# kisasexypantera94/hpfw

Measured on AMD Instinct MI355X. Metric: hashprints/sec (index) + Hamming matches/sec (search), 30 s@44.1 kHz clips, higher is better.
Workload: dtype f32 (transforms, dB) + int8 digits / int64 sums (projection); 1 GPU; configs[1]: 1000 x 30 s synthetic 44.1 kHz PCM16 clips per GPU, hashprint extraction only (CQT + dB + projection + bit pack), inputs resident in HBM; clips_per_gpu=1000, hashprints_per_clip=2320, parallelism=clips sharded over 1 GPU(s), no collective on this path

## Files before the change

### hpfw_amd/csrc/extract.hip

```cpp
#include "handle.h"

int pass_clips(hpfw_gpu *h, const DevPlan *dp, int64_t n_clips)
{
    const hpfw::HostPlan &p = dp->hp;
    size_t per_clip = (size_t)121 * p.c * 4 + (size_t)64 * std::max(p.n_frames, 1) * 4;
    if (p.bluestein)
        per_clip += 2 * hpfw::bz_plane_bytes(dp->bz, 1) + (size_t)(p.kmax - p.kmin) * 8;
    else
        per_clip += (size_t)hpfw::z_floats_per_clip(p.hq, p.n2) * 4 + (size_t)p.n1 * p.q2w * 8;
    size_t work = 0;
    for (const hpfw::CqClassDev &cd : dp->cls) work = std::max(work, hpfw::cq_big_work_bytes(cd, 1));
    per_clip += work;
    const int64_t fit = std::max<int64_t>(1, (int64_t)(((size_t)24 << 30) / per_clip));
    const int64_t cap = std::min<int64_t>(h->batch, fit), n = std::max<int64_t>(n_clips, 1);
    const int64_t passes = (n + cap - 1) / cap;
    return (int)((n + passes - 1) / passes);
}

int ensure_ws(hpfw_gpu *h, const DevPlan *dp, int nb, int ns)
{
    const hpfw::HostPlan &p = dp->hp;
    size_t work = 0;
    for (const hpfw::CqClassDev &cd : dp->cls) work = std::max(work, hpfw::cq_big_work_bytes(cd, nb));
    if (work) {
// ... 148 lines not shown
#endif
#if defined(HPFW_ROWS_STAMPS)
        dp->rows.stamps = reinterpret_cast<long long *>(g_rows_snap);
#endif
        hpfw::launch_fwd_rows2(dp->rows, dp->rows_out, yp, nb, x, s);
    }
    return check_launch("fwd_rows");
}
}

int run_front(hpfw_gpu *h, DevPlan *dp, const int16_t *d_pcm, int nb, int slot, bool finish_db, hipStream_t s)
{
    using hpfw::cf;
    const hpfw::HostPlan &p = dp->hp;
    cf *x = h->ws[1].as<cf>();
    float *mag = h->ws[2].as<float>() + (size_t)slot * 121 * p.c;
    float *mm = h->ws[4].as<float>() + (size_t)slot * 121 * hpfw::kCqMaxWaves;
    float *clipmax = h->d_clipmax.as<float>() + slot;
    int rc;
    if ((rc = run_forward(h, dp, d_pcm, nb, x, s))) return rc;
    {
        Timed t(h, K_CQ, s);
        int n_lds = 0;
        for (const hpfw::CqClassDev &cd : dp->cls) n_lds += cd.outer ? 0 : 1;
        const bool fork = h->cq_concurrent && n_lds > 1 && nb >= 4;
        Fanout fan(h, s);
        if (fork && (rc = fan.fork(hpfw_gpu::kCqSide))) return rc;
        int turn = 0;
        for (size_t ci = dp->cls.size(); ci-- > 0;) {
            const hpfw::CqClassDev &cd = dp->cls[ci];
            if (cd.outer) {
                hpfw::launch_cq_big_class(dp->cq, cd, x, nb, h->d_cqwork.as<cf>(), mag, mm, h->db_fast ? hpfw::kDbFast : hpfw::kDbSpec, s);
                continue;
            }
            const int lane = fork ? turn++ % (hpfw_gpu::kCqSide + 1) : 0;
            hpfw::launch_cq_class(dp->cq, cd, x, nb, mag, mm, h->db_fast ? hpfw::kDbFast : hpfw::kDbSpec, fan.lane(lane));
        }
        if ((rc = check_launch("cq_chirpz"))) return rc;
    }
    {
        Timed t(h, K_DB, s);
        hpfw::launch_clipmax(mm, clipmax, nb, s);
        if (finish_db) hpfw::launch_db_finish(mag, clipmax, nb, (int64_t)121 * p.c, s);
    }
    return check_launch("db");
}

int q_split(hpfw_gpu *h, int n_shifts, int64_t n_clips, int64_t c, hpfw::QSplit *qs, const hpfw::QSplit **use)
{
    *use = nullptr;
    if (n_shifts || h->q_products != 6 || !h->projection) return 0;
    const int64_t tiles = hpfw::project_q_tiles(n_clips, c);
    if (tiles <= 0) return 0;
    if (int rc = ensure(h->d_q_split, hpfw::project_q_split_bytes(tiles), h)) return rc;
    *qs = {h->d_fq_thr.as<int32_t>(), h->d_q_split.get()};
    *use = qs;
    return 0;
}

namespace {
int run_back(hpfw_gpu *h, DevPlan *dp, const void *images, int n_shifts, int ns, uint64_t *d_hp, hipStream_t s)
{
    const hpfw::HostPlan &p = dp->hp;
    const float *sdb = h->ws[2].as<float>();
    int rc;
    if (h->projection) {
        hpfw::QSplit qs;
        const hpfw::QSplit *split;
        if ((rc = q_split(h, n_shifts, ns, p.c, &qs, &split))) return rc;
        {
            Timed t(h, K_PROJECT, s);
            hpfw::launch_hashprints_q(images, n_shifts, sdb, h->d_clipmax.as<float>(), ns, p.c, d_hp, nullptr, s, split);
        }
        if (split) h->q_last_tiles = hpfw::project_q_tiles(ns, p.c);
        return check_launch("project");
    }
    float *proj = h->ws[3].as<float>();
    {
        Timed t(h, K_PROJECT, s);
        hpfw::launch_project(h->d_fpack.as<float>(), sdb, h->d_clipmax.as<float>(), ns, p.c, proj, s);
    }
    if ((rc = check_launch("project"))) return rc;
    {
        Timed t(h, K_PACK, s);
        hpfw::launch_pack(proj, ns, p.n_frames, d_hp, s);
    }
    return check_launch("delta_pack");
}

constexpr int kBackBatch = 1024;

int check_filters(const hpfw_gpu *h) { return h->has_filters ? 0 : fail(HPFW_E_NOFILTERS, "no filters: call hpfw_gpu_set_filters or hpfw_gpu_learn_filters first"); }

int check_shifts(const int32_t *shifts, int n_shifts)
{
    if (!shifts || n_shifts < 1 || n_shifts > hpfw::kMaxShifts) return fail(HPFW_E_INVALID, "shifts: 1 to 64 values");
    for (int i = 0; i < n_shifts; ++i) {
        if (shifts[i] < -(hpfw::kBins - 1) || shifts[i] > hpfw::kBins - 1) return fail(HPFW_E_INVALID, "shifts: |s| <= 120");
        for (int j = 0; j < i; ++j)
            if (shifts[j] == shifts[i]) return fail(HPFW_E_INVALID, "shifts: values must be distinct");
    }
    return 0;
}

int shift_images(hpfw_gpu *h, const int32_t *shifts, int n_shifts, hipStream_t s)
{
    std::vector<int32_t> want(shifts, shifts + n_shifts);
    if (want == h->shift_images_of) return 0;
// ... 723 lines not shown
```

### hpfw_amd/csrc/handle.h

```cpp
#pragma once
#include <hip/hip_runtime.h>

#include <algorithm>
#include <cstdio>
#include <cstdlib>
#include <cstring>
#include <condition_variable>
#include <chrono>
#include <map>
#include <memory>
#include <mutex>
#include <set>
#include <string>
#include <vector>

#include "../../include/hpfw_gpu.h"
#include "combiner.h"
#include "hip_owned.h"
#include "kernels.h"
#include "legacy_internal.h"
#include "plan.h"

using hpfw::DevBuf, hpfw::Event, hpfw::HostBuf, hpfw::Stream;

int fail(int code, const std::string &msg);

#define HIP_TRY(expr)                                                                                   \
    do {                                                                                                \
        hipError_t e_ = (expr);                                                                         \
        if (e_ != hipSuccess)                                                                           \
            return fail(HPFW_E_HIP, std::string(#expr) + ": " + hipGetErrorString(e_));                 \
    } while (0)

struct DevPlan {
    hpfw_gpu *owner = nullptr;
    std::vector<DevBuf> blocks;
    char *cur = nullptr;
    size_t left = 0;
    char *chunk_base = nullptr;
    std::vector<char> stage;
    std::vector<std::pair<size_t, size_t>> staged;
    hpfw::HostPlan hp;
    hpfw::ColsQArgs cols;
    hpfw::Rows2Out rows_out;
    hpfw::RowsArgs rows;
    hpfw::BzArgs bz;
    hpfw::CqPlanDev cq;
    std::vector<hpfw::CqClassDev> cls;
    size_t bytes = 0;
    uint64_t last_use = 0;
    ~DevPlan();
};

struct PlanTiming;

enum KernelKind { K_ROWS = 0, K_COLS, K_CQ, K_DB, K_PROJECT, K_PACK, K_SCAN, K_TOPK, K_PAIRS, K_FWD, K_COUNT };

struct TimedLaunch {
    int kind;
    Event a, b;
};

struct CallStatus {
    int rc = 0;
    std::string msg;
};

struct hpfw_gpu {
    int device = 0;
    bool has_filters = false;
    std::vector<float> filters;
    DevBuf d_fpack;
    DevBuf d_fq_image;
    DevBuf d_fq_thr, d_q_split;
    int q_products = 6;
    int64_t q_last_tiles = 0;
    int projection = 1;
    struct PlanCache {
        PlanCache();
        ~PlanCache();
        std::multimap<size_t, DevBuf> dev_pool;
        size_t dev_pool_bytes = 0;
        std::map<int64_t, std::unique_ptr<DevPlan>> plans;
        std::mutex host_mtx;
        std::condition_variable host_cv;
        std::map<int64_t, std::unique_ptr<hpfw::HostPlan>> host_ready;
        std::set<int64_t> host_seen;
        size_t plan_bytes = 0;
        uint64_t plan_clock = 0;
        uint64_t idle_clock = 0;
        std::unique_ptr<PlanTiming> plan_timing;
        Stream plan_stream;
        HostBuf pin_ring;
        size_t pin_off = 0;
        Event plan_ev;
        bool plan_ev_pending = false;
    } cache;
    unsigned conventions = 0;
    int batch = 256;
    DevBuf ws[7];
    struct Index {
        DevBuf d_db;
        std::vector<int64_t> db_off{0};
        DevBuf d_db_off;
        bool db_off_dirty = true;
        uint32_t clip_base = 0;
        DevBuf d_best, d_q_off;
        DevBuf d_qa;
        DevBuf d_gk;
        DevBuf d_topk_scratch;
        DevBuf d_shift_hits;
    } index;
    struct Learn {
        DevBuf d_cov;
        DevBuf d_cov_ws;
        DevBuf d_cov_tiles;
        int64_t cov_files = 0;
        std::map<std::vector<int>, DevBuf> cfg_fpack;
        DevBuf d_cfg_proj;
        struct CfgCov {
            DevBuf d_accum;
            DevBuf d_tiles;
            int64_t clips = 0;
        };
        std::map<std::vector<int>, CfgCov> cfg_cov;
        DevBuf d_cfg_cov_ws;
    } learn;
    struct Mel {
// ... 148 lines not shown
```

### hpfw_amd/csrc/handle.hip

```cpp
#include "handle.h"

namespace {
thread_local std::string g_err;

const char *const kKernelNames[K_COUNT] = {"fwd_rows", "fwd_cols", "cq_chirpz", "db",
                                           "project_mfma", "delta_pack", "hamming_scan", "topk", "pcm_pairs", "fwd_span"};
}

int fail(int code, const std::string &msg)
{
    g_err = msg;
    return code;
}

extern "C" {

const char *hpfw_gpu_last_error(void) { return g_err.c_str(); }
void hpfw_internal_set_error(const char *msg) { g_err = msg ? msg : ""; }
const char *hpfw_gpu_version(void) { return "hpfw-gpu 0.1 (gfx950)"; }

int hpfw_gpu_create(int device, hpfw_gpu **out)
{
    if (!out) return fail(HPFW_E_INVALID, "out is NULL");
    *out = nullptr;
    int n = 0;
    HIP_TRY(hipGetDeviceCount(&n));
    if (device < 0 || device >= n) return fail(HPFW_E_INVALID, "no such device");
    HIP_TRY(hipSetDevice(device));
    auto h = std::make_unique<hpfw_gpu>();
    h->device = device;
    if (std::getenv("HPFW_CQ_SERIAL")) h->cq_concurrent = 0;
    if (const char *e = std::getenv("HPFW_FWD_CHUNK")) h->fwd_chunk = std::max(0, atoi(e));
    if (const char *e = std::getenv("HPFW_BZ_CHUNK")) h->bz_chunk = std::max(0, atoi(e));
    if (const char *e = std::getenv("HPFW_COLS_VARIANT")) h->cols_variant = atoi(e);
    if (const char *e = std::getenv("HPFW_PRUNE")) h->prune = (unsigned)std::strtoul(e, nullptr, 0);
    if (const char *e = std::getenv("HPFW_Q_PRODUCTS")) h->q_products = atoi(e) == 9 ? 9 : 6;
    if (const char *e = std::getenv("HPFW_DB_TERM")) h->db_fast = std::strcmp(e, "spec") != 0;
    if (const char *e = std::getenv("HPFW_FWD_STREAMS")) h->fwd_streams = std::min(hpfw_gpu::kCqSide + 1, std::max(1, atoi(e)));
    if (const char *e = std::getenv("HPFW_PROJECTION"))
        h->projection = std::strcmp(e, "f32") == 0 ? 0 : 1;
    if (h->ev0.create(hipEventDefault) != hipSuccess || h->ev1.create(hipEventDefault) != hipSuccess || h->order_ev.create() != hipSuccess ||
        init_plans(h.get()) != hipSuccess)
        return fail(HPFW_E_HIP, "hipEventCreate failed");
    *out = h.release();
    return 0;
}

int hpfw_gpu_device(const hpfw_gpu *h) { return h ? h->device : -1; }

void hpfw_gpu_destroy(hpfw_gpu *h)
{
    if (!h) return;
    (void)hipSetDevice(h->device);
    (void)hipDeviceSynchronize();
    delete h;
}

int hpfw_gpu_set_filters(hpfw_gpu *h, const float *f)
{
    if (!h || !f) return fail(HPFW_E_INVALID, "null argument");
    HIP_TRY(hipSetDevice(h->device));
    std::vector<float> packed((size_t)hpfw::kFilters * hpfw::kFrame);
    hpfw::pack_filters_for_mfma(f, packed.data());
    if (!h->d_fpack) HIP_TRY(h->d_fpack.alloc(packed.size() * 4));
    HIP_TRY(hipMemcpy(h->d_fpack.get(), packed.data(), packed.size() * 4, hipMemcpyHostToDevice));
    std::vector<int8_t> image;
    std::vector<int32_t> fq_thr;
    hpfw::pack_filters_q(f, image, &fq_thr);
    if (!h->d_fq_image) HIP_TRY(h->d_fq_image.alloc(image.size()));
    HIP_TRY(hipMemcpy(h->d_fq_image.get(), image.data(), image.size(), hipMemcpyHostToDevice));
    if (!h->d_fq_thr) HIP_TRY(h->d_fq_thr.alloc(fq_thr.size() * 4));
    HIP_TRY(hipMemcpy(h->d_fq_thr.get(), fq_thr.data(), fq_thr.size() * 4, hipMemcpyHostToDevice));
    h->shift_images_of.clear();
    h->filters.assign(f, f + (size_t)hpfw::kFilters * hpfw::kFrame);
    h->has_filters = true;
    return 0;
}

int hpfw_gpu_get_filters(hpfw_gpu *h, float *out)
{
    if (!h || !out) return fail(HPFW_E_INVALID, "null argument");
    if (!h->has_filters) return fail(HPFW_E_NOFILTERS, "no filters: call hpfw_gpu_set_filters or hpfw_gpu_learn_filters first");
    std::memcpy(out, h->filters.data(), h->filters.size() * sizeof(float));
    return 0;
}

int hpfw_gpu_set_projection(hpfw_gpu *h, int mode)
{
    if (!h || (mode != 0 && mode != 1)) return fail(HPFW_E_INVALID, "projection mode must be 0 (f32 chain) or 1 (fixed point)");
    h->projection = mode;
    return 0;
}

int hpfw_gpu_get_projection(hpfw_gpu *h) { return h ? h->projection : -1; }

int hpfw_gpu_set_conventions(hpfw_gpu *h, unsigned flags)
{
    if (!h || flags > hpfw::kConvAll) return fail(HPFW_E_INVALID, "unknown convention flag");
    HIP_TRY(hipSetDevice(h->device));
    if (flags != h->conventions) {
        HIP_TRY(hipDeviceSynchronize());
        clear_plans(h);
    }
    h->conventions = flags;
    return 0;
}

int hpfw_gpu_set_batch(hpfw_gpu *h, int clips)
{
    if (!h || clips < 0 || clips > 4096) return fail(HPFW_E_INVALID, "batch out of range");
    h->batch = clips == 0 ? 256 : clips;
    return 0;
}

int hpfw_gpu_timer_start(hpfw_gpu *h, void *stream)
{
    if (!h) return fail(HPFW_E_INVALID, "null handle");
    HIP_TRY(hipEventRecord(h->ev0.get(), (hipStream_t)stream));
    return 0;
}

int hpfw_gpu_timer_stop(hpfw_gpu *h, void *stream, float *ms)
{
    if (!h || !ms) return fail(HPFW_E_INVALID, "null argument");
    HIP_TRY(hipEventRecord(h->ev1.get(), (hipStream_t)stream));
// ... 41 lines not shown
```

### hpfw_amd/csrc/k_project_q.hip

```cpp
#include <algorithm>
#include <cmath>
#include <cstdint>
#include <cstdlib>
#include <vector>

#include "kernels.h"

namespace hpfw {

extern __shared__ __align__(16) unsigned char smem_raw[];

typedef int v4i __attribute__((ext_vector_type(4)));
typedef int v16i __attribute__((ext_vector_type(16)));

constexpr int kQThreads = 256;
constexpr int kQTileN = 128;
constexpr int kQCols = kQTileN + kCtx - 1;
constexpr int kQPitch = 160;
constexpr int kQChunks = 8;
constexpr int kQUnit = 48;
constexpr int kQSlabBytes = kQChunks * kQPitch * kQUnit;
constexpr int kQStepBytes = 3 * 64 * 16;
constexpr int kQSteps = 2 * kCtx;
constexpr int kQLdsBytes = kQSlabBytes + kQTileN * 4 * 2;
constexpr float kQScale = 98304.0f;
constexpr int kQCap = 128;
constexpr unsigned kQRedo = 0xffffffffu;
constexpr int kQLdsBytes6 = kQLdsBytes + 16;

__device__ __forceinline__ unsigned q_digit_bytes(int u) { return ((unsigned)u + 0x808080u) ^ 0x808080u; }

__device__ __forceinline__ int q_fixed(float s)
{
    return (int)__builtin_rintf(__builtin_fminf(__builtin_fmaxf(s, -80.0f), 0.0f) * kQScale);
}

template <bool FROM_T, bool SHIFTED, int NP>
__device__ __forceinline__ void hashprint_q_tile(const unsigned t, const v4i *__restrict__ fq_images, const float *__restrict__ sdb,
                                                 const float *__restrict__ tmax, int c, int nhp, int n_tiles_x, uint64_t *__restrict__ hp,
                                                 long long *__restrict__ dbg, int n_images, const int *__restrict__ thr,
                                                 unsigned *__restrict__ counts, unsigned short *__restrict__ seg)
{
    static_assert(NP == 9 || (NP == 6 && !SHIFTED), "six products: the extraction's unshifted image only");
    unsigned char *slab = smem_raw;
    unsigned short *parts = reinterpret_cast<unsigned short *>(smem_raw + kQSlabBytes);
    unsigned *n_open = reinterpret_cast<unsigned *>(smem_raw + kQLdsBytes);
    const int tid = threadIdx.x, lane = tid & 63, wave = tid >> 6;
    const int kg = lane >> 4, cl = lane & 15;
    const int clip = t / n_tiles_x;
    const int n0 = (t - clip * n_tiles_x) * kQTileN;
    if (NP == 6 && tid == 0) *n_open = 0;
#if defined(HPFW_Q_STAMPS)
    long long st[6];
    st[0] = __builtin_amdgcn_s_memtime();
#define Q_STAMP(k) st[k] = __builtin_amdgcn_s_memtime()
#else
#define Q_STAMP(k) ((void)0)
#endif
    const float *S = sdb + (int64_t)clip * kBins * c;
    const float ref = FROM_T ? tmax[clip] : 0.0f;
    const v4i *img = fq_images + (size_t)wave * kQSteps * (kQStepBytes / 16) + lane;
    v4i a[3][3];
#pragma unroll
    for (int d = 0; d < 3; ++d) {
        a[0][d] = img[d * 64];
        a[1][d] = img[(kQStepBytes / 16) + d * 64];
    }
    constexpr int kUnits = (kQChunks * kQCols + kQThreads - 1) / kQThreads;
    unsigned any_digit = 0;
#pragma unroll 1
    for (int r0 = 0; r0 < kUnits; r0 += 2) {
        float va[2][16], vb[2][16];
#pragma unroll
        for (int rr = 0; rr < 2; ++rr) {
            const int unit = tid + (r0 + rr) * kQThreads;
            const int q = unit / kQCols, col = unit - q * kQCols;
            const int gc = n0 + col;
            const bool in = r0 + rr < kUnits && unit < kQChunks * kQCols && gc + kLag < c;
#pragma unroll
            for (int e = 0; e < 16; ++e) {
                const int bin = 16 * q + e;
                const bool ok = in && bin < kBins;
                const unsigned idx = ok ? (unsigned)(bin * c + gc) : 0u;
                va[rr][e] = S[idx];
                vb[rr][e] = S[idx + kLag];
            }
        }
#pragma unroll
        for (int rr = 0; rr < 2; ++rr) {
            const int unit = tid + (r0 + rr) * kQThreads;
            const int q = unit / kQCols, col = unit - q * kQCols;
            const bool in = r0 + rr < kUnits && unit < kQChunks * kQCols && n0 + col + kLag < c;
#pragma unroll
            for (int e = 0; e < 16; ++e) {
                const bool ok = in && 16 * q + e < kBins;
                va[rr][e] = ok ? va[rr][e] : 0.0f;
                vb[rr][e] = ok ? vb[rr][e] : 0.0f;
            }
        }
#pragma unroll
        for (int rr = 0; rr < 2; ++rr) {
            const int unit = tid + (r0 + rr) * kQThreads;
            if (r0 + rr >= kUnits || unit >= kQChunks * kQCols) break;
            const int q = unit / kQCols, col = unit - q * kQCols;
            unsigned w0[4] = {0, 0, 0, 0}, w1[4] = {0, 0, 0, 0}, w2[4] = {0, 0, 0, 0};
#pragma unroll
            for (int e = 0; e < 16; ++e) {
                float xa = va[rr][e], xb = vb[rr][e];
                if (FROM_T) {
                    xa -= ref;
                    xb -= ref;
                }
                const unsigned d = q_digit_bytes(q_fixed(xa) - q_fixed(xb));
                w0[e >> 2] |= (d & 255u) << (8 * (e & 3));
                w1[e >> 2] |= ((d >> 8) & 255u) << (8 * (e & 3));
                w2[e >> 2] |= ((d >> 16) & 255u) << (8 * (e & 3));
            }
            v4i *dst = reinterpret_cast<v4i *>(slab + (size_t)(q * kQPitch + col) * kQUnit);
            dst[0] = v4i{(int)w0[0], (int)w0[1], (int)w0[2], (int)w0[3]};
            dst[1] = v4i{(int)w1[0], (int)w1[1], (int)w1[2], (int)w1[3]};
            dst[2] = v4i{(int)w2[0], (int)w2[1], (int)w2[2], (int)w2[3]};
            if (NP == 6)
                any_digit |= w0[0] | w0[1] | w0[2] | w0[3] | w1[0] | w1[1] | w1[2] | w1[3] | w2[0] | w2[1] | w2[2] | w2[3];
        }
    }
    Q_STAMP(1);
    if (NP == 6) {
        if (!__syncthreads_or((int)(any_digit != 0))) {
            if (tid < kQTileN && n0 + tid < nhp) hp[(int64_t)clip * nhp + n0 + tid] = ~0ull;
            if (tid == 0) counts[t] = 0;
            return;
        }
    } else {
        __syncthreads();
    }
    Q_STAMP(2);
    const int n_tiles = min(8, (nhp - n0 + 15) / 16);
    const unsigned char *bl = slab + (size_t)(kg * kQPitch + cl) * kQUnit;
    int im = 0;
#pragma unroll 1
    do {
        if (SHIFTED && im > 0) {
            __syncthreads();
            img += (size_t)4 * kQSteps * kQStepBytes / 16;
#pragma unroll
            for (int d = 0; d < 3; ++d) {
                a[0][d] = img[d * 64];
                a[1][d] = img[(kQStepBytes / 16) + d * 64];
            }
        }
        v4i acc[8][5];
#pragma unroll
        for (int f = 0; f < 8; ++f)
#pragma unroll
            for (int cls = 0; cls < 5; ++cls) acc[f][cls] = v4i{0, 0, 0, 0};
        auto step = [&](int s, const v4i (&aw)[3]) {
            const unsigned char *bs = bl + (size_t)((4 * (s & 1)) * kQPitch + (s >> 1)) * kQUnit;
            v4i nb0, nb1, nb2;
            {
                const v4i *bu = reinterpret_cast<const v4i *>(bs);
                nb0 = bu[0], nb1 = bu[1], nb2 = bu[2];
            }
#pragma unroll
            for (int f = 0; f < 8; ++f) {
                if (f < n_tiles) {
                    const v4i b0 = nb0, b1 = nb1, b2 = nb2;
                    if (f + 1 < 8) {
                        const v4i *bu = reinterpret_cast<const v4i *>(bs + (size_t)(16 * (f + 1)) * kQUnit);
                        nb0 = bu[0], nb1 = bu[1], nb2 = bu[2];
                    }
                    __builtin_amdgcn_sched_barrier(0);
                    if (NP == 9) {
                        acc[f][0] = __builtin_amdgcn_mfma_i32_16x16x64_i8(aw[0], b0, acc[f][0], 0, 0, 0);
                        acc[f][1] = __builtin_amdgcn_mfma_i32_16x16x64_i8(aw[0], b1, acc[f][1], 0, 0, 0);
                    }
                    acc[f][2] = __builtin_amdgcn_mfma_i32_16x16x64_i8(aw[0], b2, acc[f][2], 0, 0, 0);
                    acc[f][3] = __builtin_amdgcn_mfma_i32_16x16x64_i8(aw[1], b2, acc[f][3], 0, 0, 0);
                    acc[f][4] = __builtin_amdgcn_mfma_i32_16x16x64_i8(aw[2], b2, acc[f][4], 0, 0, 0);
                    if (NP == 9) acc[f][1] = __builtin_amdgcn_mfma_i32_16x16x64_i8(aw[1], b0, acc[f][1], 0, 0, 0);
                    acc[f][2] = __builtin_amdgcn_mfma_i32_16x16x64_i8(aw[1], b1, acc[f][2], 0, 0, 0);
                    acc[f][3] = __builtin_amdgcn_mfma_i32_16x16x64_i8(aw[2], b1, acc[f][3], 0, 0, 0);
                    acc[f][2] = __builtin_amdgcn_mfma_i32_16x16x64_i8(aw[2], b0, acc[f][2], 0, 0, 0);
                }
            }
        };
        auto load_a = [&](int s, v4i (&aw)[3]) {
            if (s < kQSteps) {
#pragma unroll
                for (int d = 0; d < 3; ++d) aw[d] = img[(size_t)s * (kQStepBytes / 16) + d * 64];
            }
        };
        if (n_tiles > 0) {
#pragma unroll 1
            for (int s = 0; s < kQSteps - 1; s += 3) {
                load_a(s + 2, a[2]);
                step(s, a[0]);
                load_a(s + 3, a[0]);
                step(s + 1, a[1]);
                load_a(s + 4, a[1]);
                step(s + 2, a[2]);
            }
            step(kQSteps - 1, a[0]);
        }
        Q_STAMP(3);
        v4i th = v4i{-1, -1, -1, -1};
        if (NP == 6) th = *reinterpret_cast<const v4i *>(thr + 16 * wave + 4 * kg);
#pragma unroll
        for (int f = 0; f < 8; ++f) {
            const int n = n0 + 16 * f + cl;
            (void)n;
            unsigned bits = 0;
#pragma unroll
            for (int reg = 0; reg < 4; ++reg) {
                const int row = 4 * kg + reg;
                long long v = acc[f][4][reg];
#pragma unroll
                for (int cls = 3; cls >= (NP == 9 ? 0 : 2); --cls) v = v * 256 + acc[f][cls][reg];
                bits |= (unsigned)(v >= 0) << (15 - row);
                if (NP == 6 && f < n_tiles && n < nhp && (v < 0 ? -v : v) <= (long long)th[reg]) {
                    const unsigned pos = atomicAdd(n_open, 1u);
                    if (pos < (unsigned)kQCap) seg[(size_t)t * kQCap + pos] = (unsigned short)(((16 * wave + row) << 7) | (16 * f + cl));
                }
#if !defined(HPFW_Q_STAMPS)
                if (!SHIFTED && dbg && f < n_tiles && n < nhp) dbg[((int64_t)clip * kFilters + 16 * wave + row) * nhp + n] = v;
#endif
            }
            bits |= (unsigned)__shfl_xor((int)bits, 16);
            bits |= (unsigned)__shfl_xor((int)bits, 32);
            if (kg == 0) parts[(16 * f + cl) * 4 + wave] = (unsigned short)bits;
        }
        Q_STAMP(4);
        __syncthreads();
        if (tid < kQTileN && n0 + tid < nhp) {
            const unsigned short *p = parts + tid * 4;
            hp[((int64_t)clip * (SHIFTED ? n_images : 1) + im) * nhp + n0 + tid] =
                ((uint64_t)p[0] << 48) | ((uint64_t)p[1] << 32) | ((uint64_t)p[2] << 16) | (uint64_t)p[3];
        }
        if (NP == 6 && tid == 0) counts[t] = *n_open <= (unsigned)kQCap ? *n_open : kQRedo;
    } while (SHIFTED && ++im < n_images);
#if defined(HPFW_Q_STAMPS)
    Q_STAMP(5);
    if (dbg && tid == 0) {
        for (int k = 0; k < 6; ++k) dbg[(int64_t)t * 8 + k] = st[k];
        dbg[(int64_t)t * 8 + 6] = __builtin_amdgcn_s_getreg((15 << 11) | 4);
        dbg[(int64_t)t * 8 + 7] = blockIdx.x;
    }
#endif
}

__device__ __forceinline__ unsigned q_tile_of_workgroup()
{
    const unsigned per_xcd = (gridDim.x + 7) / 8;
    return (blockIdx.x & 7) * per_xcd + (blockIdx.x >> 3);
}

template <bool FROM_T, bool SHIFTED>
__global__ __launch_bounds__(kQThreads, 2) void hashprint_q_kernel(const v4i *__restrict__ fq_images, const float *__restrict__ sdb,
                                                                   const float *__restrict__ tmax, int c, int nhp, int n_tiles_x, int n_clips,
                                                                   uint64_t *__restrict__ hp, long long *__restrict__ dbg, int n_images)
{
    const unsigned t = q_tile_of_workgroup();
    if (t >= (unsigned)(n_tiles_x * n_clips)) return;
    hashprint_q_tile<FROM_T, SHIFTED, 9>(t, fq_images, sdb, tmax, c, nhp, n_tiles_x, hp, dbg, n_images, nullptr, nullptr, nullptr);
}

template <bool FROM_T>
__global__ __launch_bounds__(kQThreads, 2) void hashprint_q6_kernel(const v4i *__restrict__ fq_image, const float *__restrict__ sdb,
                                                                    const float *__restrict__ tmax, int c, int nhp, int n_tiles_x, int n_clips,
                                                                    uint64_t *__restrict__ hp, const int *__restrict__ thr,
                                                                    unsigned *__restrict__ counts, unsigned short *__restrict__ seg)
{
    const unsigned t = q_tile_of_workgroup();
    if (t >= (unsigned)(n_tiles_x * n_clips)) return;
    hashprint_q_tile<FROM_T, false, 6>(t, fq_image, sdb, tmax, c, nhp, n_tiles_x, hp, nullptr, 1, thr, counts, seg);
}

template <bool FROM_T>
__global__ __launch_bounds__(kQThreads, 2) void hashprint_q_fixup_kernel(const v4i *__restrict__ fq_image, const int *__restrict__ fq32,
                                                                         const float *__restrict__ sdb, const float *__restrict__ tmax, int c,
                                                                         int nhp, int n_tiles_x, int n_clips, uint64_t *__restrict__ hp,
                                                                         const unsigned *__restrict__ counts,
                                                                         const unsigned short *__restrict__ seg)
{
    const int lane = threadIdx.x & 63, wave = threadIdx.x >> 6;
    const unsigned total = (unsigned)(n_tiles_x * n_clips);
    for (unsigned t = blockIdx.x; t < total; t += gridDim.x) {
        const unsigned cnt = counts[t];
        if (cnt == 0) continue;
        if (cnt == kQRedo) {
            __syncthreads();
            hashprint_q_tile<FROM_T, false, 9>(t, fq_image, sdb, tmax, c, nhp, n_tiles_x, hp, nullptr, 1, nullptr, nullptr, nullptr);
            continue;
        }
        const int clip = t / n_tiles_x;
        const int n0 = (t - clip * n_tiles_x) * kQTileN;
        const float *S = sdb + (int64_t)clip * kBins * c;
        const float ref = FROM_T ? tmax[clip] : 0.0f;
        for (unsigned e = wave; e < cnt; e += kQThreads / 64) {
            const unsigned entry = seg[(size_t)t * kQCap + e];
            const int r = entry >> 7, n = n0 + (int)(entry & 127u);
            const int *frow = fq32 + r * kFrame;
            long long sum = 0;
#pragma unroll 2
            for (int k = lane; k < kFrame; k += 64) {
                const int bin = k / kCtx, idx = bin * c + n + (k - bin * kCtx);
                float xa = S[idx], xb = S[idx + kLag];
                if (FROM_T) {
                    xa -= ref;
                    xb -= ref;
                }
                sum += (long long)frow[k] * (long long)(q_fixed(xa) - q_fixed(xb));
            }
#pragma unroll
            for (int m = 32; m >= 1; m >>= 1) sum += __shfl_xor(sum, m);
            if (lane == 0) {
                unsigned long long *w = reinterpret_cast<unsigned long long *>(hp + (int64_t)clip * nhp + n);
                const unsigned long long bit = 1ull << (63 - r);
                if (((*w & bit) != 0) != (sum >= 0)) atomicXor(w, bit);
            }
        }
    }
}

__global__ __launch_bounds__(256) void shift_filter_images_kernel(const unsigned char *__restrict__ base, ShiftList shifts,
                                                                  v4i *__restrict__ out)
{
    constexpr int kUnits = 4 * kQSteps * kQStepBytes / 16;
    const int u = blockIdx.x * 256 + threadIdx.x;
    if (u >= kUnits) return;
    const int s = shifts.s[blockIdx.y];
    const int l = u & 63, i = (u >> 6) % 3, ws = u / 192;
    const int step = ws % kQSteps, w = ws / kQSteps, t = step >> 1, p = step & 1;
    unsigned wd[4] = {0, 0, 0, 0};
#pragma unroll
    for (int e = 0; e < 16; ++e) {
        const int b = 64 * p + 16 * (l >> 4) + e, src = b - s;
        if (b < kBins && src >= 0 && src < kBins) {
            const unsigned char v = base[((size_t)w * kQSteps + 2 * t + (src >> 6)) * kQStepBytes + ((size_t)i * 64 + (l & 15) + 16 * ((src >> 4) & 3)) * 16 +
                                         (src & 15)];
            wd[e >> 2] |= (unsigned)v << (8 * (e & 3));
        }
    }
    out[(size_t)blockIdx.y * kUnits + u] = v4i{(int)wd[0], (int)wd[1], (int)wd[2], (int)wd[3]};
}

void pack_filters_q(const float *f, std::vector<int8_t> &image, std::vector<int32_t> *fq_thr)
{
    std::vector<int32_t> fq((size_t)kFilters * kFrame);
    for (int r = 0; r < kFilters; ++r) {
        float m = 0.0f;
        for (int k = 0; k < kFrame; ++k) m = std::fmax(m, std::fabs(f[(size_t)k * kFilters + r]));
        const int e = m > 0.0f ? 21 - std::ilogb(m) : 0;
        for (int k = 0; k < kFrame; ++k) fq[(size_t)r * kFrame + k] = (int32_t)std::rint(std::ldexp(f[(size_t)k * kFilters + r], e));
    }
    if (fq_thr) {
        fq_thr->assign(fq.begin(), fq.end());
        for (int r = 0; r < kFilters; ++r) {
            int64_t s0 = 0, s1 = 0;
            for (int k = 0; k < kFrame; ++k) {
                const int u = fq[(size_t)r * kFrame + k];
                const int d0 = ((u + 128) & 255) - 128, u1 = (u - d0) >> 8, d1 = ((u1 + 128) & 255) - 128;
                s0 += std::abs(d0);
                s1 += std::abs(d1);
            }
            const int64_t lmax = 128 * (s0 + 256 * (s0 + s1));
            fq_thr->push_back(lmax > 0 ? (int32_t)(lmax >> 16) : -1);
        }
    }
    image.assign((size_t)4 * kQSteps * kQStepBytes, 0);
    for (int w = 0; w < 4; ++w)
        for (int t = 0; t < kCtx; ++t)
            for (int p = 0; p < 2; ++p)
                for (int l = 0; l < 64; ++l)
                    for (int e = 0; e < 16; ++e) {
                        const int bin = 64 * p + 16 * (l >> 4) + e;
                        if (bin >= kBins) continue;
                        const int u = fq[(size_t)(16 * w + (l & 15)) * kFrame + bin * kCtx + t];
                        const int d0 = ((u + 128) & 255) - 128, u1 = (u - d0) >> 8, d1 = ((u1 + 128) & 255) - 128, d2 = (u1 - d1) >> 8;
                        const int d[3] = {d0, d1, d2};
                        for (int i = 0; i < 3; ++i)
                            image[((size_t)w * kQSteps + (2 * t + p)) * kQStepBytes + ((size_t)i * 64 + l) * 16 + e] = (int8_t)d[i];
                    }
}

#if defined(HPFW_Q_STAMPS)
static long long *g_q_stamps = nullptr;
extern "C" void hpfw_gpu_debug_set_q_stamps(void *d) { g_q_stamps = static_cast<long long *>(d); }
#endif

size_t project_q_image_bytes() { return (size_t)4 * kQSteps * kQStepBytes; }
size_t project_q_split_bytes(int64_t tiles) { return (size_t)tiles * (4 + (size_t)kQCap * 2); }
int64_t project_q_tiles(int64_t n_clips, int64_t c)
{
    const int64_t nhp = c - (kCtx - 1) - kLag;
    return nhp > 0 ? n_clips * ((nhp + kQTileN - 1) / kQTileN) : 0;
}

void launch_hashprints_q(const void *d_images, int n_shifts, const float *d_db, const float *d_tmax, int n_clips, int c, uint64_t *d_hp,
                         long long *d_dbg, hipStream_t s, const QSplit *split)
{
    static PerDeviceOnce attr_set;
    if (attr_set.need()) {
        for (const void *k : {reinterpret_cast<const void *>(hashprint_q_kernel<true, false>), reinterpret_cast<const void *>(hashprint_q_kernel<false, false>),
                              reinterpret_cast<const void *>(hashprint_q_kernel<true, true>), reinterpret_cast<const void *>(hashprint_q_kernel<false, true>)})
            (void)hipFuncSetAttribute(k, hipFuncAttributeMaxDynamicSharedMemorySize, kQLdsBytes);
        for (const void *k : {reinterpret_cast<const void *>(hashprint_q6_kernel<true>), reinterpret_cast<const void *>(hashprint_q6_kernel<false>),
                              reinterpret_cast<const void *>(hashprint_q_fixup_kernel<true>), reinterpret_cast<const void *>(hashprint_q_fixup_kernel<false>)})
            (void)hipFuncSetAttribute(k, hipFuncAttributeMaxDynamicSharedMemorySize, kQLdsBytes6);
        attr_set.mark();
    }
    const int nhp = c - (kCtx - 1) - kLag;
    if (nhp <= 0 || n_clips <= 0 || n_shifts < 0) return;
#if defined(HPFW_Q_STAMPS)
    if (!d_dbg) d_dbg = g_q_stamps;
#endif
    const int tiles = (nhp + kQTileN - 1) / kQTileN;
    const dim3 grid(8 * (unsigned)(((int64_t)tiles * n_clips + 7) / 8));
    if (split && n_shifts == 0 && !d_dbg) {
        const int *fq32 = split->d_fq_thr, *thr = fq32 + (size_t)kFilters * kFrame;
        unsigned *counts = static_cast<unsigned *>(split->d_work);
        unsigned short *seg = reinterpret_cast<unsigned short *>(counts + (size_t)tiles * n_clips);
        hipLaunchKernelGGL(d_tmax ? hashprint_q6_kernel<true> : hashprint_q6_kernel<false>, grid, dim3(kQThreads), kQLdsBytes6, s,
                           static_cast<const v4i *>(d_images), d_db, d_tmax, c, nhp, tiles, n_clips, d_hp, thr, counts, seg);
        const unsigned fix = (unsigned)std::min<int64_t>((int64_t)tiles * n_clips, 2048);
        hipLaunchKernelGGL(d_tmax ? hashprint_q_fixup_kernel<true> : hashprint_q_fixup_kernel<false>, dim3(fix), dim3(kQThreads), kQLdsBytes6, s,
                           static_cast<const v4i *>(d_images), fq32, d_db, d_tmax, c, nhp, tiles, n_clips, d_hp, counts, seg);
        return;
    }
    auto k = n_shifts > 0 ? (d_tmax ? hashprint_q_kernel<true, true> : hashprint_q_kernel<false, true>)
                          : (d_tmax ? hashprint_q_kernel<true, false> : hashprint_q_kernel<false, false>);
    hipLaunchKernelGGL(k, grid, dim3(kQThreads), kQLdsBytes, s, static_cast<const v4i *>(d_images), d_db, d_tmax, c, nhp, tiles, n_clips,
                       d_hp, d_dbg, n_shifts);
}

void launch_shift_filter_images(const void *d_fq_image, const ShiftList &shifts, void *d_images, hipStream_t s)
{
    constexpr int kUnits = 4 * kQSteps * kQStepBytes / 16;
    hipLaunchKernelGGL(shift_filter_images_kernel, dim3((kUnits + 255) / 256, shifts.n), dim3(256), 0, s,
                       static_cast<const unsigned char *>(d_fq_image), shifts, static_cast<v4i *>(d_images));
}

}
```

### hpfw_amd/csrc/kernels.h

```cpp
#pragma once
#include <cmath>
#include <cstdint>
#include <vector>
#include <atomic>
#include <hip/hip_runtime.h>
#include <stdint.h>

#include "../../include/hpfw_gpu.h"
#include "device_math.h"
#include "fft_lds.h"
#include "fft_rows.h"
#include "streams_plan.h"
#include "xcorr_plan.h"

namespace hpfw {

struct PerDeviceOnce {
    std::atomic<uint64_t> done{0};
    static uint64_t bit()
    {
        int dev = 0;
        (void)hipGetDevice(&dev);
        return 1ull << (dev & 63);
    }
// ... 125 lines not shown
    int kmin, nk;
    int xn1, xw, xq0;
    int64_t xclip;
    unsigned long long xmagic;
    HPFW_DEVICE_MEMBER XsView view(const cf *x, int clip) const { return XsView{x + (int64_t)clip * xclip, xn1, xw, xq0, xmagic}; }
    int c;
    const int *start;
    const int *lg;
    const int64_t *g_off;
    const cf *g;
    const cf *g2;
    const int64_t *g2_off;
    const int *q2a, *nq2;
    const unsigned *nq2_magic;
    int rows_min;
};

struct CqWindowBands {
    double scale[121];
    int hann_den[121];
};
void launch_cq_windows(const CqPlanDev &c, const CqWindowBands &b, int64_t big_m, int lg_max, cf *d_g, hipStream_t s);
void launch_cq_windows_rows(const CqPlanDev &c, int n1, int max_entries, cf *d_g2, hipStream_t s);

void launch_fwd_cols_q(const ColsQArgs &a, const int16_t *d_pcm, int64_t clip_samples, int n_clips, float *d_z, hipStream_t s);
size_t fwd_rows_lds_bytes(const RowsArgs &a);
void launch_fwd_rows2(const RowsArgs &a, const Rows2Out &o, const float *d_z, int n_clips, cf *d_x, hipStream_t s);
void launch_gather_bins(const CqPlanDev &cp, const cf *d_x, int n_clips, cf *d_out, hipStream_t s);
size_t bz_plane_bytes(const BzArgs &bz, int n_clips);
void launch_bz_pack_stages(const BzArgs &bz, const cf *d_tw_n1, float *d_apack1, float *d_apack3, hipStream_t s);
void launch_bz_pack_coefficients(int n1, int k1_first, int k1_count, const cf *d_tw_n1, int n_tiles, float *d_apack, hipStream_t s);
void launch_bz_make_tables(const RowsArgs &rows, const BzArgs &bz, int64_t n, float *d_b, float *d_y, hipStream_t s);
void launch_bz_cols_first(const BzArgs &bz, const int16_t *d_pcm, int64_t n, int n_clips, float *d_out, hipStream_t s);
void launch_bz_rows_both(const RowsArgs &rows, const BzArgs &bz, const float *d_in, int n_clips, float *d_out, hipStream_t s);
void launch_bz_cols_last(const BzArgs &bz, const float *d_in, int n_clips, cf *d_x, hipStream_t s);
constexpr int kCqMaxWaves = 16;
enum DbMode { kDbNone = 0, kDbSpec = 1, kDbFast = 2 };
void launch_cq_class(const CqPlanDev &cp, const CqClassDev &cc, const cf *d_x, int n_clips,
                     float *d_mag, float *d_wavemax, int db_mode, hipStream_t s);
size_t cq_big_work_bytes(const CqClassDev &cc, int n_clips);
void launch_cq_big_class(const CqPlanDev &cp, const CqClassDev &cc, const cf *d_x, int n_clips, cf *d_work, float *d_mag,
                         float *d_wavemax, int db_mode, hipStream_t s);
void launch_clipmax(const float *d_wavemax, float *d_clipmax, int n_clips, hipStream_t s);
void launch_db_finish(float *d_t, const float *d_clipmax, int n_clips, int64_t per_clip, hipStream_t s);
void launch_magmax(const float *d_mag, int n_clips, int c, float *d_wavemax, hipStream_t s);
void launch_db(const float *d_mag, const float *d_wavemax, float *d_clipmax, int n_clips, int64_t per_clip,
               float *d_db, bool fast, hipStream_t s);
void launch_db_term_sweep(uint32_t first, uint64_t count, unsigned long long *d_out, hipStream_t s);
void launch_project(const float *d_fpack, const float *d_db, const float *d_tmax, int n_clips, int c,
                    float *d_proj, hipStream_t s);
void launch_pack(const float *d_proj, int n_clips, int nf, uint64_t *d_hp, hipStream_t s);
size_t project_q_image_bytes();
struct QSplit {
    const int32_t *d_fq_thr;
    void *d_work;
};
size_t project_q_split_bytes(int64_t tiles);
int64_t project_q_tiles(int64_t n_clips, int64_t c);
void pack_filters_q(const float *f_colmajor, std::vector<int8_t> &image, std::vector<int32_t> *fq_thr = nullptr);
void launch_hashprints_q(const void *d_images, int n_shifts, const float *d_db, const float *d_tmax, int n_clips, int c, uint64_t *d_hp,
                         long long *d_dbg, hipStream_t s, const QSplit *split = nullptr);
constexpr int kMaxShifts = 64;
struct ShiftList {
    int n;
    int s[kMaxShifts];
};
void launch_shift_filter_images(const void *d_fq_image, const ShiftList &shifts, void *d_images, hipStream_t s);
constexpr int kMaxTempos = 64;
struct TempoList {
    int n;
    int32_t step[kMaxTempos];
};
inline int32_t tempo_step(float rho) { return (int32_t)std::rint(65536.0 / (double)rho); }
inline int64_t tempo_columns(int64_t c, int32_t step) { return (c - 1) * 65536 / step + 1; }
void launch_tempo_scale(const float *d_db, int n_clips, int64_t c, const TempoList &tl, int64_t ct, float *d_out, hipStream_t s);

struct CfgArgs {
    int rows, context, lag, filters;
    const float *fpack;
};
size_t cfg_fpack_floats(int rows, int context, int filters);
void pack_cfg_filters(int rows, int context, int filters, const float *f_colmajor, float *fpack);
size_t project_cfg_lds_bytes(const CfgArgs &a);
void launch_project_cfg(const CfgArgs &a, const float *d_s, const int *d_cols, int n_clips, int64_t stride, float *d_proj,
                        int64_t proj_stride, hipStream_t s);
void launch_pack_cfg(const CfgArgs &a, const float *d_proj, const int *d_cols, int n_clips, int64_t stride, int64_t proj_stride,
                     void *d_hp, int64_t hp_stride, hipStream_t s);

bool cov_cfg_supported(const CfgArgs &a);
int cov_cfg_tile_count(int kt);
void cov_cfg_tile_list(int kt, int *xy );
size_t cov_cfg_workspace_bytes(const CfgArgs &a, int n_clips);
void launch_cov_cfg(const CfgArgs &a, const float *d_s, const int *d_cols, int n_clips, int64_t stride, const int *d_tiles,
                    float *d_ws, float *d_accum, hipStream_t s);

int cov_tile_count();
void cov_tile_list(int *xy );
size_t cov_workspace_bytes(int n_clips, int c);
void launch_cov(const float *d_db, int n_clips, int c, const int *d_tiles, float *d_ws, float *d_accum, hipStream_t s);
int top_eigenvectors(const float *cov, int n, int m, float *out, double *evals);

void pack_filters_for_mfma(const float *filters_colmajor, float *fpack );

constexpr int kMelFrame = 4410, kMelHop = 441, kMelBins = 2206, kMelBands = 33;
int mel_frames(int64_t n_samples);
size_t mel_work_bytes(int64_t n_samples, int n_clips);
void launch_mel(const RowsArgs &rows, const float *d_win, const float *d_cpack, const int16_t *d_pcm, int64_t n, int n_clips,
                int64_t *d_blk, int *d_pos, int *d_count, float *d_pmax, float *d_work, float *d_out, bool db_fast, hipStream_t s);
void launch_mel_kept_frames(const int16_t *d_pcm, int64_t n, int n_clips, int64_t *d_blk, int *d_pos, int *d_count,
                            int32_t *d_frames, int64_t stride, hipStream_t s);

void launch_xcorr(const int16_t *d_pcm, const XcJob *d_jobs, int64_t n_jobs, const XcItem *d_mfma, int64_t n_mfma,
// ... 66 lines not shown
```

Baseline: 276.8 million hashprints/s.

## Fuse six-product projection fixup into the main kernel using LDS entry list

The six-product quantized projection previously wrote near-threshold entries to a global segment list, and a separate fixup kernel recomputed them. It now keeps the list in LDS and resolves each listed entry in the same workgroup: it recomputes the exact value from the digit slab with sdot4 and flips the sign bit when needed. Overflowing tiles fall back to an in-kernel nine-product redo. The old two-launch path stays available via HPFW_Q_FIXUP=launch. This removes the second launch and the global segment traffic, at the cost of extra LDS and possible tail imbalance inside the fused kernel.

```diff
diff --git a/hpfw_amd/csrc/extract.hip b/hpfw_amd/csrc/extract.hip
--- a/hpfw_amd/csrc/extract.hip
+++ b/hpfw_amd/csrc/extract.hip
@@ -224,8 +224,8 @@
     if (n_shifts || h->q_products != 6 || !h->projection) return 0;
     const int64_t tiles = hpfw::project_q_tiles(n_clips, c);
     if (tiles <= 0) return 0;
-    if (int rc = ensure(h->d_q_split, hpfw::project_q_split_bytes(tiles), h)) return rc;
-    *qs = {h->d_fq_thr.as<int32_t>(), h->d_q_split.get()};
+    if (int rc = ensure(h->d_q_split, hpfw::project_q_split_bytes(tiles, h->q_fixup_launch), h)) return rc;
+    *qs = {h->d_q_thr.as<int32_t>(), h->d_q_split.get(), h->q_fixup_launch ? h->d_fq32.as<int32_t>() : nullptr};
     *use = qs;
     return 0;
 }
diff --git a/hpfw_amd/csrc/handle.h b/hpfw_amd/csrc/handle.h
--- a/hpfw_amd/csrc/handle.h
+++ b/hpfw_amd/csrc/handle.h
@@ -72,8 +72,9 @@
     std::vector<float> filters;
     DevBuf d_fpack;
     DevBuf d_fq_image;
-    DevBuf d_fq_thr, d_q_split;
+    DevBuf d_q_thr, d_fq32, d_q_split;
     int q_products = 6;
+    bool q_fixup_launch = false;
     int64_t q_last_tiles = 0;
     int projection = 1;
     struct PlanCache {
diff --git a/hpfw_amd/csrc/handle.hip b/hpfw_amd/csrc/handle.hip
--- a/hpfw_amd/csrc/handle.hip
+++ b/hpfw_amd/csrc/handle.hip
@@ -35,6 +35,7 @@
     if (const char *e = std::getenv("HPFW_COLS_VARIANT")) h->cols_variant = atoi(e);
     if (const char *e = std::getenv("HPFW_PRUNE")) h->prune = (unsigned)std::strtoul(e, nullptr, 0);
     if (const char *e = std::getenv("HPFW_Q_PRODUCTS")) h->q_products = atoi(e) == 9 ? 9 : 6;
+    if (const char *e = std::getenv("HPFW_Q_FIXUP")) h->q_fixup_launch = std::strcmp(e, "launch") == 0;
     if (const char *e = std::getenv("HPFW_DB_TERM")) h->db_fast = std::strcmp(e, "spec") != 0;
     if (const char *e = std::getenv("HPFW_FWD_STREAMS")) h->fwd_streams = std::min(hpfw_gpu::kCqSide + 1, std::max(1, atoi(e)));
     if (const char *e = std::getenv("HPFW_PROJECTION"))
@@ -65,12 +66,16 @@
     if (!h->d_fpack) HIP_TRY(h->d_fpack.alloc(packed.size() * 4));
     HIP_TRY(hipMemcpy(h->d_fpack.get(), packed.data(), packed.size() * 4, hipMemcpyHostToDevice));
     std::vector<int8_t> image;
-    std::vector<int32_t> fq_thr;
-    hpfw::pack_filters_q(f, image, &fq_thr);
+    std::vector<int32_t> thr, fq32;
+    hpfw::pack_filters_q(f, image, &thr, h->q_fixup_launch ? &fq32 : nullptr);
     if (!h->d_fq_image) HIP_TRY(h->d_fq_image.alloc(image.size()));
     HIP_TRY(hipMemcpy(h->d_fq_image.get(), image.data(), image.size(), hipMemcpyHostToDevice));
-    if (!h->d_fq_thr) HIP_TRY(h->d_fq_thr.alloc(fq_thr.size() * 4));
-    HIP_TRY(hipMemcpy(h->d_fq_thr.get(), fq_thr.data(), fq_thr.size() * 4, hipMemcpyHostToDevice));
+    if (!h->d_q_thr) HIP_TRY(h->d_q_thr.alloc(thr.size() * 4));
+    HIP_TRY(hipMemcpy(h->d_q_thr.get(), thr.data(), thr.size() * 4, hipMemcpyHostToDevice));
+    if (h->q_fixup_launch) {
+        if (!h->d_fq32) HIP_TRY(h->d_fq32.alloc(fq32.size() * 4));
+        HIP_TRY(hipMemcpy(h->d_fq32.get(), fq32.data(), fq32.size() * 4, hipMemcpyHostToDevice));
+    }
     h->shift_images_of.clear();
     h->filters.assign(f, f + (size_t)hpfw::kFilters * hpfw::kFrame);
     h->has_filters = true;
diff --git a/hpfw_amd/csrc/k_project_q.hip b/hpfw_amd/csrc/k_project_q.hip
--- a/hpfw_amd/csrc/k_project_q.hip
+++ b/hpfw_amd/csrc/k_project_q.hip
@@ -27,6 +27,7 @@
 constexpr int kQCap = 128;
 constexpr unsigned kQRedo = 0xffffffffu;
 constexpr int kQLdsBytes6 = kQLdsBytes + 16;
+constexpr int kQLdsBytes6f = kQLdsBytes6 + kQCap * 2;
 
 __device__ __forceinline__ unsigned q_digit_bytes(int u) { return ((unsigned)u + 0x808080u) ^ 0x808080u; }
 
@@ -35,16 +36,52 @@
     return (int)__builtin_rintf(__builtin_fminf(__builtin_fmaxf(s, -80.0f), 0.0f) * kQScale);
 }
 
-template <bool FROM_T, bool SHIFTED, int NP>
+__device__ __forceinline__ long long q_value_from_digits(const v4i *__restrict__ fq_image, const unsigned char *slab, int r, int nl, int lane)
+{
+    constexpr int kPairs = 4 * kQSteps;
+    v4i fa[3][3], sb[3][3];
+#pragma unroll
+    for (int k = 0; k < 3; ++k) {
+        const int pair = min(lane + 64 * k, kPairs - 1);
+        const int s = pair >> 2, g = pair & 3;
+        const v4i *fu = fq_image + ((size_t)(r >> 4) * kQSteps + s) * (kQStepBytes / 16) + (r & 15) + 16 * g;
+        const v4i *su = reinterpret_cast<const v4i *>(slab + (size_t)((4 * (s & 1) + g) * kQPitch + nl + (s >> 1)) * kQUnit);
+#pragma unroll
+        for (int d = 0; d < 3; ++d) {
+            fa[k][d] = fu[d * 64];
+            sb[k][d] = su[d];
+        }
+    }
+    if (lane + 128 >= kPairs) sb[2][0] = sb[2][1] = sb[2][2] = v4i{0, 0, 0, 0};
+    int acc[5] = {0, 0, 0, 0, 0};
+#pragma unroll
+    for (int k = 0; k < 3; ++k)
+#pragma unroll
+        for (int i = 0; i < 3; ++i)
+#pragma unroll
+            for (int j = 0; j < 3; ++j)
+#pragma unroll
+                for (int w = 0; w < 4; ++w) acc[i + j] = __builtin_amdgcn_sdot4(fa[k][i][w], sb[k][j][w], acc[i + j], false);
+    long long v = acc[4];
+#pragma unroll
+    for (int cls = 3; cls >= 0; --cls) v = v * 256 + acc[cls];
+#pragma unroll
+    for (int m = 32; m >= 1; m >>= 1) v += __shfl_xor(v, m);
+    return v;
+}
+
+template <bool FROM_T, bool SHIFTED, int NP, bool FUSED = false, bool STAGED = false>
 __device__ __forceinline__ void hashprint_q_tile(const unsigned t, const v4i *__restrict__ fq_images, const float *__restrict__ sdb,
                                                  const float *__restrict__ tmax, int c, int nhp, int n_tiles_x, uint64_t *__restrict__ hp,
                                                  long long *__restrict__ dbg, int n_images, const int *__restrict__ thr,
                                                  unsigned *__restrict__ counts, unsigned short *__restrict__ seg)
 {
     static_assert(NP == 9 || (NP == 6 && !SHIFTED), "six products: the extraction's unshifted image only");
+    static_assert((!FUSED || NP == 6) && (!STAGED || (NP == 9 && !SHIFTED)), "FUSED: six products; STAGED: its nine-product redo");
     unsigned char *slab = smem_raw;
     unsigned short *parts = reinterpret_cast<unsigned short *>(smem_raw + kQSlabBytes);
     unsigned *n_open = reinterpret_cast<unsigned *>(smem_raw + kQLdsBytes);
+    unsigned short *list = reinterpret_cast<unsigned short *>(smem_raw + kQLdsBytes6);
     const int tid = threadIdx.x, lane = tid & 63, wave = tid >> 6;
     const int kg = lane >> 4, cl = lane & 15;
     const int clip = t / n_tiles_x;
@@ -69,7 +106,7 @@
     constexpr int kUnits = (kQChunks * kQCols + kQThreads - 1) / kQThreads;
     unsigned any_digit = 0;
 #pragma unroll 1
-    for (int r0 = 0; r0 < kUnits; r0 += 2) {
+    for (int r0 = STAGED ? kUnits : 0; r0 < kUnits; r0 += 2) {
         float va[2][16], vb[2][16];
 #pragma unroll
         for (int rr = 0; rr < 2; ++rr) {
@@ -125,7 +162,8 @@
         }
     }
     Q_STAMP(1);
-    if (NP == 6) {
+    if (STAGED) {
+    } else if (NP == 6) {
         if (!__syncthreads_or((int)(any_digit != 0))) {
             if (tid < kQTileN && n0 + tid < nhp) hp[(int64_t)clip * nhp + n0 + tid] = ~0ull;
             if (tid == 0) counts[t] = 0;
@@ -219,7 +257,8 @@
                 bits |= (unsigned)(v >= 0) << (15 - row);
                 if (NP == 6 && f < n_tiles && n < nhp && (v < 0 ? -v : v) <= (long long)th[reg]) {
                     const unsigned pos = atomicAdd(n_open, 1u);
-                    if (pos < (unsigned)kQCap) seg[(size_t)t * kQCap + pos] = (unsigned short)(((16 * wave + row) << 7) | (16 * f + cl));
+                    if (pos < (unsigned)kQCap)
+                        (FUSED ? list : seg + (size_t)t * kQCap)[pos] = (unsigned short)(((16 * wave + row) << 7) | (16 * f + cl));
                 }
 #if !defined(HPFW_Q_STAMPS)
                 if (!SHIFTED && dbg && f < n_tiles && n < nhp) dbg[((int64_t)clip * kFilters + 16 * wave + row) * nhp + n] = v;
@@ -231,6 +270,27 @@
         }
         Q_STAMP(4);
         __syncthreads();
+        if (FUSED) {
+            const unsigned cnt = *n_open;
+            if (cnt > (unsigned)kQCap) {
+                if (tid == 0) counts[t] = kQRedo;
+                hashprint_q_tile<FROM_T, false, 9, false, true>(t, fq_images, sdb, tmax, c, nhp, n_tiles_x, hp, nullptr, 1, nullptr, nullptr, nullptr);
+                return;
+            }
+            if (cnt > 0) {
+                for (unsigned e = (unsigned)__builtin_amdgcn_readfirstlane(wave); e < cnt; e += kQThreads / 64) {
+                    const int entry = __builtin_amdgcn_readfirstlane((int)list[e]);
+                    const int r = entry >> 7, nl = entry & 127;
+                    const long long d = q_value_from_digits(fq_images, slab, r, nl, lane);
+                    if (lane == 0) {
+                        unsigned *w = reinterpret_cast<unsigned *>(parts) + nl * 2 + (r >> 5);
+                        const unsigned bit = 1u << (16 * ((r >> 4) & 1) + 15 - (r & 15));
+                        if (((*static_cast<volatile unsigned *>(w) & bit) != 0) != (d >= 0)) atomicXor(w, bit);
+                    }
+                }
+                __syncthreads();
+            }
+        }
         if (tid < kQTileN && n0 + tid < nhp) {
             const unsigned short *p = parts + tid * 4;
             hp[((int64_t)clip * (SHIFTED ? n_images : 1) + im) * nhp + n0 + tid] =
@@ -268,7 +328,18 @@
 __global__ __launch_bounds__(kQThreads, 2) void hashprint_q6_kernel(const v4i *__restrict__ fq_image, const float *__restrict__ sdb,
                                                                     const float *__restrict__ tmax, int c, int nhp, int n_tiles_x, int n_clips,
                                                                     uint64_t *__restrict__ hp, const int *__restrict__ thr,
-                                                                    unsigned *__restrict__ counts, unsigned short *__restrict__ seg)
+                                                                    unsigned *__restrict__ counts)
+{
+    const unsigned t = q_tile_of_workgroup();
+    if (t >= (unsigned)(n_tiles_x * n_clips)) return;
+    hashprint_q_tile<FROM_T, false, 6, true>(t, fq_image, sdb, tmax, c, nhp, n_tiles_x, hp, nullptr, 1, thr, counts, nullptr);
+}
+
+template <bool FROM_T>
+__global__ __launch_bounds__(kQThreads, 2) void hashprint_q6_listed_kernel(const v4i *__restrict__ fq_image, const float *__restrict__ sdb,
+                                                                           const float *__restrict__ tmax, int c, int nhp, int n_tiles_x,
+                                                                           int n_clips, uint64_t *__restrict__ hp, const int *__restrict__ thr,
+                                                                           unsigned *__restrict__ counts, unsigned short *__restrict__ seg)
 {
     const unsigned t = q_tile_of_workgroup();
     if (t >= (unsigned)(n_tiles_x * n_clips)) return;
@@ -344,7 +415,7 @@
     out[(size_t)blockIdx.y * kUnits + u] = v4i{(int)wd[0], (int)wd[1], (int)wd[2], (int)wd[3]};
 }
 
-void pack_filters_q(const float *f, std::vector<int8_t> &image, std::vector<int32_t> *fq_thr)
+void pack_filters_q(const float *f, std::vector<int8_t> &image, std::vector<int32_t> *thr, std::vector<int32_t> *fq32)
 {
     std::vector<int32_t> fq((size_t)kFilters * kFrame);
     for (int r = 0; r < kFilters; ++r) {
@@ -353,8 +424,9 @@
         const int e = m > 0.0f ? 21 - std::ilogb(m) : 0;
         for (int k = 0; k < kFrame; ++k) fq[(size_t)r * kFrame + k] = (int32_t)std::rint(std::ldexp(f[(size_t)k * kFilters + r], e));
     }
-    if (fq_thr) {
-        fq_thr->assign(fq.begin(), fq.end());
+    if (fq32) *fq32 = fq;
+    if (thr) {
+        thr->clear();
         for (int r = 0; r < kFilters; ++r) {
             int64_t s0 = 0, s1 = 0;
             for (int k = 0; k < kFrame; ++k) {
@@ -364,7 +436,7 @@
                 s1 += std::abs(d1);
             }
             const int64_t lmax = 128 * (s0 + 256 * (s0 + s1));
-            fq_thr->push_back(lmax > 0 ? (int32_t)(lmax >> 16) : -1);
+            thr->push_back(lmax > 0 ? (int32_t)(lmax >> 16) : -1);
         }
     }
     image.assign((size_t)4 * kQSteps * kQStepBytes, 0);
@@ -389,7 +461,7 @@
 #endif
 
 size_t project_q_image_bytes() { return (size_t)4 * kQSteps * kQStepBytes; }
-size_t project_q_split_bytes(int64_t tiles) { return (size_t)tiles * (4 + (size_t)kQCap * 2); }
+size_t project_q_split_bytes(int64_t tiles, bool segments) { return (size_t)tiles * (4 + (segments ? (size_t)kQCap * 2 : 0)); }
 int64_t project_q_tiles(int64_t n_clips, int64_t c)
 {
     const int64_t nhp = c - (kCtx - 1) - kLag;
@@ -404,9 +476,11 @@
         for (const void *k : {reinterpret_cast<const void *>(hashprint_q_kernel<true, false>), reinterpret_cast<const void *>(hashprint_q_kernel<false, false>),
                               reinterpret_cast<const void *>(hashprint_q_kernel<true, true>), reinterpret_cast<const void *>(hashprint_q_kernel<false, true>)})
             (void)hipFuncSetAttribute(k, hipFuncAttributeMaxDynamicSharedMemorySize, kQLdsBytes);
-        for (const void *k : {reinterpret_cast<const void *>(hashprint_q6_kernel<true>), reinterpret_cast<const void *>(hashprint_q6_kernel<false>),
+        for (const void *k : {reinterpret_cast<const void *>(hashprint_q6_listed_kernel<true>), reinterpret_cast<const void *>(hashprint_q6_listed_kernel<false>),
                               reinterpret_cast<const void *>(hashprint_q_fixup_kernel<true>), reinterpret_cast<const void *>(hashprint_q_fixup_kernel<false>)})
             (void)hipFuncSetAttribute(k, hipFuncAttributeMaxDynamicSharedMemorySize, kQLdsBytes6);
+        for (const void *k : {reinterpret_cast<const void *>(hashprint_q6_kernel<true>), reinterpret_cast<const void *>(hashprint_q6_kernel<false>)})
+            (void)hipFuncSetAttribute(k, hipFuncAttributeMaxDynamicSharedMemorySize, kQLdsBytes6f);
         attr_set.mark();
     }
     const int nhp = c - (kCtx - 1) - kLag;
@@ -417,10 +491,15 @@
     const int tiles = (nhp + kQTileN - 1) / kQTileN;
     const dim3 grid(8 * (unsigned)(((int64_t)tiles * n_clips + 7) / 8));
     if (split && n_shifts == 0 && !d_dbg) {
-        const int *fq32 = split->d_fq_thr, *thr = fq32 + (size_t)kFilters * kFrame;
+        const int *fq32 = split->d_fq32, *thr = split->d_thr;
         unsigned *counts = static_cast<unsigned *>(split->d_work);
+        if (!fq32) {
+            hipLaunchKernelGGL(d_tmax ? hashprint_q6_kernel<true> : hashprint_q6_kernel<false>, grid, dim3(kQThreads), kQLdsBytes6f, s,
+                               static_cast<const v4i *>(d_images), d_db, d_tmax, c, nhp, tiles, n_clips, d_hp, thr, counts);
+            return;
+        }
         unsigned short *seg = reinterpret_cast<unsigned short *>(counts + (size_t)tiles * n_clips);
-        hipLaunchKernelGGL(d_tmax ? hashprint_q6_kernel<true> : hashprint_q6_kernel<false>, grid, dim3(kQThreads), kQLdsBytes6, s,
+        hipLaunchKernelGGL(d_tmax ? hashprint_q6_listed_kernel<true> : hashprint_q6_listed_kernel<false>, grid, dim3(kQThreads), kQLdsBytes6, s,
                            static_cast<const v4i *>(d_images), d_db, d_tmax, c, nhp, tiles, n_clips, d_hp, thr, counts, seg);
         const unsigned fix = (unsigned)std::min<int64_t>((int64_t)tiles * n_clips, 2048);
         hipLaunchKernelGGL(d_tmax ? hashprint_q_fixup_kernel<true> : hashprint_q_fixup_kernel<false>, dim3(fix), dim3(kQThreads), kQLdsBytes6, s,
diff --git a/hpfw_amd/csrc/kernels.h b/hpfw_amd/csrc/kernels.h
--- a/hpfw_amd/csrc/kernels.h
+++ b/hpfw_amd/csrc/kernels.h
@@ -201,12 +201,13 @@
 void launch_pack(const float *d_proj, int n_clips, int nf, uint64_t *d_hp, hipStream_t s);
 size_t project_q_image_bytes();
 struct QSplit {
-    const int32_t *d_fq_thr;
+    const int32_t *d_thr;
     void *d_work;
-};
-size_t project_q_split_bytes(int64_t tiles);
+    const int32_t *d_fq32;
+};
+size_t project_q_split_bytes(int64_t tiles, bool segments);
 int64_t project_q_tiles(int64_t n_clips, int64_t c);
-void pack_filters_q(const float *f_colmajor, std::vector<int8_t> &image, std::vector<int32_t> *fq_thr = nullptr);
+void pack_filters_q(const float *f_colmajor, std::vector<int8_t> &image, std::vector<int32_t> *thr = nullptr, std::vector<int32_t> *fq32 = nullptr);
 void launch_hashprints_q(const void *d_images, int n_shifts, const float *d_db, const float *d_tmax, int n_clips, int c, uint64_t *d_hp,
                          long long *d_dbg, hipStream_t s, const QSplit *split = nullptr);
 constexpr int kMaxShifts = 64;
```

Result: faster. 286.8 million hashprints/s, median of 6 (+3.6%).
